# iden3/rapidsnark-old

Hardware: AMD Instinct MI355X
Metric: Groth16 proofs/sec (higher is better)
Workload: dtype i64 (v_mad_i64_i32 column sums over 9x29-bit signed limbs, BN254 Fr/Fq)

## Files before the change

rapidsnark-old_amd/csrc/kernels.hpp:

```cpp
#pragma once
#include <hip/hip_runtime.h>
#include <stdint.h>
#include "field.hpp"
#include "curve.hpp"

namespace zk {

void launch_fr_mul_vec(Fr *out, const Fr *a, const Fr *b, uint64_t n, hipStream_t s);
void launch_fq_mul_vec(Fq *out, const Fq *a, const Fq *b, uint64_t n, hipStream_t s);

struct CsrDev {
    const uint32_t *rowptr;
    const uint32_t *col;
    const Fr *val;
};
void launch_spmv_abc(Fr *a, Fr *b, Fr *c, CsrDev csr, const Fr *wtns, uint32_t n, hipStream_t s, uint32_t vectors = 1, uint64_t abc_stride = 0,
                     uint64_t wtns_stride = 0);
void launch_csr_build(uint32_t *rowptr, uint32_t *col, Fr *val, uint32_t *cursor, uint32_t *err, const uint8_t *records,
                      uint64_t nCoefs, uint32_t n, uint32_t nVars, uint32_t row_lo, uint32_t row_hi, hipStream_t s);
void launch_exclusive_scan_u32(uint32_t *out, const uint32_t *counts, uint32_t total, hipStream_t s);

struct TwEntry {
    uint32_t l[12];
};
// ... 23 lines not shown
void launch_ntt_build_tables(TwEntry *fwd, TwEntry *inv, Fr *coset, Fr *ninv, uint32_t logn, hipStream_t s);
#define NTT_FULL 0xffffffffu
void launch_ntt_dif_inverse(Fr *data, uint64_t stride_elems, uint32_t batch, const NttTables &t, hipStream_t s, uint32_t local_logn = NTT_FULL);
void launch_ntt_dit_forward(Fr *data, uint64_t stride_elems, uint32_t batch, const NttTables &t, hipStream_t s, const Fr *premul = nullptr,
                            uint32_t local_logn = NTT_FULL);
void launch_ntt_cross(bool inverse, const Fr *xb, uint64_t in_src_stride, uint64_t in_poly_stride, Fr *const out_base[8],
                      uint64_t out_poly_stride, uint64_t out_offset, uint32_t batch,
                      const NttTables &t, uint32_t log_shards, uint32_t rank, hipStream_t s);
void launch_chunk_scatter(Fr *const xb_of_gpu[8], const Fr *blockdata, uint32_t batch, uint32_t logn, uint32_t log_shards, uint32_t rank,
                          hipStream_t s);
void launch_chunk_pack(Fr *packed, const Fr *blockdata, uint32_t batch, uint32_t logn, uint32_t log_shards, hipStream_t s);
void launch_chunk_unpack(Fr *blockdata, const Fr *packed, uint32_t batch, uint32_t logn, uint32_t log_shards, hipStream_t s);
void launch_fr_to_internal(Fr *x, uint64_t n, int times, hipStream_t s);
void launch_fr_from_internal(Fr *x, uint64_t n, hipStream_t s);
void launch_fr_scale_by_table(Fr *data, uint64_t stride_elems, uint32_t batch, const Fr *table, uint64_t n, hipStream_t s);
void launch_fr_scale_const(Fr *data, const Fr *k, uint64_t n, hipStream_t s);
void launch_bitrev_permute(Fr *data, uint32_t logn, hipStream_t s);
void launch_abc_to_h(Fr *h, const Fr *a, const Fr *b, const Fr *c, uint64_t n, hipStream_t s, uint32_t vectors = 1, uint64_t abc_stride = 0);

struct MsmPlan {
    uint32_t c;
    uint32_t W;
    uint32_t nbuckets;
    uint32_t sets;
    uint32_t precomp;
    uint32_t batch;
    uint32_t batch_n;
};
MsmPlan make_msm_plan(uint64_t n, uint32_t window_bits, uint32_t precomp = 0, uint32_t batch = 1);
inline uint32_t msm_table_rows(const MsmPlan &p) { return p.precomp ? (p.W + p.precomp - 1) / p.precomp : 1u; }

struct MsmSortSizes {
    uint64_t counts_u32, starts_u32, offsets_u32, entries_u32;
    uint64_t codes_u32, lo_u16, val_u32, bin_counts_u32, bin_starts_u32;
};
struct MsmSortBufs {
    uint32_t *offsets, *entries;
    uint32_t *counts, *starts;
    uint32_t *codes, *val, *bin_counts, *bin_starts;
    uint16_t *lo;
};
MsmSortSizes msm_sort_sizes(uint64_t n, MsmPlan p);
uint32_t msm_scan_extra_words(uint32_t total);
void launch_msm_sort(const MsmSortBufs &b, const Fr *scalars, uint64_t n, MsmPlan p, hipStream_t s);
void launch_msm_precomp_g1(G1Affine *table, G1XYZZ *tmp, Fq *pref, uint64_t n, MsmPlan p, hipStream_t s);
void launch_msm_precomp_g2(G2Affine *table, G2XYZZ *tmp, Fq2 *pref, uint64_t n, MsmPlan p, hipStream_t s);
struct alignas(16) G1Acc {
    int32_t l[36];
};
struct alignas(16) G2Acc {
    int32_t l[72];
};
uint64_t msm_accum_workspace_slots(uint64_t max_entries);
struct AccumTail {
    hipStream_t stream = nullptr;
    hipEvent_t l1_done = nullptr;
    bool buckets_zeroed = false;
    uint32_t chunk_min = 0;
    uint32_t chunk_max = 0;
};
struct AccumBatch {
    uint32_t n;
    const void *points[3];
    uint32_t idx_min[3], idx_sub[3];
    uint64_t bucket_stride, ws_stride;
    uint32_t gather_mask;
};
void launch_msm_accum_g1_batch(G1Acc *buckets, const uint32_t *offsets, const uint32_t *entries, const AccumBatch &batch, uint32_t total_buckets,
                               uint64_t max_entries, G1Acc *ws_part, uint32_t *ws_key, uint32_t *ws_flag, hipStream_t s, hipEvent_t *ev = nullptr,
                               AccumTail tail = AccumTail());
void launch_msm_accum_g1(G1Acc *buckets, const uint32_t *offsets, const uint32_t *entries, const G1Affine *points,
                         uint32_t idx_min, uint32_t idx_sub, uint32_t total_buckets, uint64_t max_entries,
// ... 22 lines not shown
```

rapidsnark-old_amd/csrc/msm.hip:

```cpp
#include <stdlib.h>
#include "kernels.hpp"
#include "hipcheck.hpp"
#include "common.hpp"
#include "field29.hpp"
#include "curve29.hpp"
#include <string.h>

namespace zk {

#define REDUCE_CHUNK 16u
#define REDUCE_THREADS 256u

MsmPlan make_msm_plan(uint64_t n, uint32_t window_bits, uint32_t precomp, uint32_t batch) {
    if (precomp > 2) throw std::invalid_argument("table mode: 0 (as in the zkey), 1 (a row per window) or 2 (a row per second window)");
    MsmPlan p;
    uint32_t lg = 0;
    while ((1ull << (lg + 1)) <= n) lg++;
    uint32_t c = window_bits;
    if (precomp) {
        if (c == 0) {
            c = lg > 2 ? lg - 2 : 2;
            if (lg == 20) c = 19;
            if (lg == 21) c = 20;
            if (batch > 1) c++;
            if (c > 20) c = 20;
        }
        if (c > 22) c = 22;
    } else {
        if (c == 0) c = lg > 6 ? lg - 6 : 2;
        if (c > 16) c = 16;
    }
    if (c < 2) c = 2;
    p.c = c;
    p.W = (256 + c - 1) / c;
    {
        const uint32_t W255 = (255 + c - 1) / c;
        if (W255 < p.W) {
            const uint32_t sh = (W255 - 1) * c;
// ... 151 lines not shown
        int32_t w[36];
        load36(w, p->l);
        return unpack36(w);
    }
    __device__ __forceinline__ static void store(G1Acc *p, const XYZZ<R> &v) {
        int32_t w[36];
        pack36(w, v.x, v.y, v.zz, v.zzz);
        store36(p->l, w);
    }
    __device__ __forceinline__ static void store256(G1XYZZ *p, const XYZZ<R> &v) { store_xyzz_mont256(p, v); }
};
template <> struct LaneModel<Fq2> {
    static constexpr uint32_t LPE = 2;
    typedef Fq2s R;
    typedef G2Acc Mem;
    __device__ __forceinline__ static XYZZ<R> load(const G2Acc *p) {
        int32_t w[36];
        load36(w, p->l + 36 * (threadIdx.x & 1u));
        const XYZZ<Fq29> t = unpack36(w);
        return XYZZ<R>{R{t.x}, R{t.y}, R{t.zz}, R{t.zzz}};
    }
    __device__ __forceinline__ static void store(G2Acc *p, const XYZZ<R> &v) {
        int32_t w[36];
        pack36(w, v.x.v, v.y.v, v.zz.v, v.zzz.v);
        store36(p->l + 36 * (threadIdx.x & 1u), w);
    }
    __device__ __forceinline__ static void store256(G2XYZZ *p, const XYZZ<R> &v) {
        Fq *c = reinterpret_cast<Fq *>(p) + (threadIdx.x & 1u);
        Reg<Fq>::store256(c, v.x.v); Reg<Fq>::store256(c + 2, v.y.v); Reg<Fq>::store256(c + 4, v.zz.v); Reg<Fq>::store256(c + 6, v.zzz.v);
    }
};
#define ACCMEM typename LaneModel<F>::Mem

#define CODE32_ZERO 0x7FFFFFFFu
#ifndef SORT_THREADS
#define SORT_THREADS 1024u
#endif

__global__ __launch_bounds__(256) void k_msm_digits(uint32_t *digits, const Fr *scalars, uint64_t n, MsmPlan p) {
    ZK_CHAIN_PRIO();
    uint64_t st = (uint64_t)gridDim.x * blockDim.x;
    const uint32_t c = p.c, W = p.W;
    const uint32_t mask = (1u << c) - 1u, half = 1u << (c - 1);
    const uint32_t set_stride = p.precomp == 1 ? 0u : p.nbuckets, set_mask = p.precomp == 2 ? 1u : 0xffffffffu;
    for (uint64_t i = (uint64_t)blockIdx.x * blockDim.x + threadIdx.x; i < n; i += st) {
        Fr s = load_el(scalars + i);
        const uint32_t vec_base = p.batch > 1 ? (uint32_t)(i / p.batch_n) * p.nbuckets : 0u;
        for (int k = 0; k < 6; k++) {
            Fr d;
            u32 bw = 0;
#pragma unroll
            for (int j = 0; j < 8; j++) d.v[j] = subb(s.v[j], FrParams::P[j], bw);
            if (bw) break;
            s = d;
        }
        uint64_t buf = 0;
        uint32_t nb = 0, w = 0, carry = 0;
        auto emit = [&](uint32_t raw) {
            uint32_t d = raw + carry;
            const bool neg = d >= half;
            carry = neg ? 1u : 0u;
            uint32_t mag = neg ? (1u << c) - d : d;
            uint32_t code = mag ? ((mag - 1u + (w & set_mask) * set_stride + vec_base) | (neg ? 0x80000000u : 0u)) : CODE32_ZERO;
            digits[(uint64_t)w * n + i] = code;
            w++;
        };
#pragma unroll
        for (int k = 0; k < 8; k++) {
            buf |= (uint64_t)s.v[k] << nb;
            nb += 32;
            while (nb >= c && w + 1 < W) {
                emit((uint32_t)buf & mask);
                buf >>= c;
                nb -= c;
            }
        }
        emit((uint32_t)buf & mask);
    }
}

__global__ __launch_bounds__(256) void k_msm_compact_offsets(uint32_t *offsets, const uint32_t *starts, uint32_t total, uint32_t slices) {
    ZK_CHAIN_PRIO();
    uint32_t k = blockIdx.x * blockDim.x + threadIdx.x;
    if (k <= total) offsets[k] = starts[(uint64_t)k * slices];
}

#define BIN_MAX 256u

__global__ __launch_bounds__(SORT_THREADS) void k_bin_count(uint32_t *bin_counts, const uint32_t *codes, uint64_t total, uint32_t nbins,
                                                            uint32_t nblocks, uint32_t shift, uint32_t span) {
    ZK_CHAIN_PRIO();
    __shared__ uint32_t hist[BIN_MAX];
    if (threadIdx.x < BIN_MAX) hist[threadIdx.x] = 0;
    __syncthreads();
    const uint64_t base = (uint64_t)blockIdx.x * span;
    for (uint32_t k = threadIdx.x; k < span; k += SORT_THREADS) {
        uint64_t i = base + k;
        if (i < total) {
            uint32_t code = codes[i];
            if ((code & 0x7FFFFFFFu) != CODE32_ZERO) atomicAdd(&hist[(code & 0x7FFFFFFFu) >> shift], 1u);
        }
    }
    __syncthreads();
    if (threadIdx.x < nbins) bin_counts[(uint64_t)threadIdx.x * nblocks + blockIdx.x] = hist[threadIdx.x];
}

#define BIN_ITEMS 8u
__global__ __launch_bounds__(SORT_THREADS) void k_bin_scatter(uint16_t *lo, uint32_t *val, const uint32_t *bin_starts, const uint32_t *codes,
                                                              uint64_t total, uint32_t nbins, uint32_t nblocks, uint32_t shift, uint32_t span, uint64_t n,
                                                              uint32_t set_shift, uint32_t batch_n, uint32_t tstride) {
    ZK_CHAIN_PRIO();
    extern __shared__ uint32_t smem[];
    uint32_t *cnt = smem;
    uint32_t *gdelta = smem + BIN_MAX;
    uint32_t *st_dst = smem + 2 * BIN_MAX;
    uint32_t *st_val = st_dst + span;
    uint16_t *st_lo = (uint16_t *)(st_val + span);
    const uint32_t tid = threadIdx.x;
    if (tid < BIN_MAX) cnt[tid] = 0;
    __syncthreads();
    const uint64_t base = (uint64_t)blockIdx.x * span;
    const uint32_t lomask = (1u << shift) - 1u;
    const uint64_t w_base = tstride > 1 && n ? base / n : 0, r_base = tstride > 1 && n ? base - w_base * n : 0;
    uint32_t code[BIN_ITEMS], rank[BIN_ITEMS];
#pragma unroll
    for (uint32_t k = 0; k < BIN_ITEMS; k++) {
        uint64_t i = base + (uint64_t)k * SORT_THREADS + tid;
        code[k] = i < total ? codes[i] : CODE32_ZERO;
    }
#pragma unroll
    for (uint32_t k = 0; k < BIN_ITEMS; k++) {
        uint32_t mag = code[k] & 0x7FFFFFFFu;
        rank[k] = mag != CODE32_ZERO ? atomicAdd(&cnt[mag >> shift], 1u) : 0u;
    }
    __syncthreads();
    if (tid < 64) {
        uint32_t c0 = cnt[4 * tid], c1 = cnt[4 * tid + 1], c2 = cnt[4 * tid + 2], c3 = cnt[4 * tid + 3];
        uint32_t sum = c0 + c1 + c2 + c3, x = sum;
#pragma unroll
        for (int d = 1; d < 64; d <<= 1) {
            uint32_t y = __shfl_up(x, d);
            if (tid >= (uint32_t)d) x += y;
        }
        uint32_t off = x - sum;
        uint32_t o[4] = {off, off + c0, off + c0 + c1, off + c0 + c1 + c2};
#pragma unroll
        for (int q = 0; q < 4; q++) {
            uint32_t bin = 4 * tid + q;
            cnt[bin] = o[q];
            gdelta[bin] = bin < nbins ? bin_starts[(uint64_t)bin * nblocks + blockIdx.x] - o[q] : 0u;
        }
        if (tid == 63) smem[2 * BIN_MAX + 2 * span + span / 2] = x;
    }
    __syncthreads();
#pragma unroll
    for (uint32_t k = 0; k < BIN_ITEMS; k++) {
        uint32_t mag = code[k] & 0x7FFFFFFFu;
        if (mag != CODE32_ZERO) {
            uint32_t bin = mag >> shift, slot = cnt[bin] + rank[k];
            uint64_t i = base + (uint64_t)k * SORT_THREADS + tid - (uint64_t)(set_shift < 32 ? mag >> set_shift : 0u) * n;
            if (tstride > 1) {
                uint64_t w = w_base, r = r_base + (uint64_t)k * SORT_THREADS + tid;
                while (n && r >= n) { r -= n; w++; }
                i = (w / tstride) * n + r;
            }
            if (batch_n) {
                const uint64_t j = i / n, r = (i % n) % batch_n;
                i = j * batch_n + r;
            }
            st_dst[slot] = slot + gdelta[bin];
            st_val[slot] = (uint32_t)i | (code[k] & 0x80000000u);
            st_lo[slot] = (uint16_t)(mag & lomask);
        }
    }
    __syncthreads();
    const uint32_t kept = smem[2 * BIN_MAX + 2 * span + span / 2];
    for (uint32_t sidx = tid; sidx < kept; sidx += SORT_THREADS) {
        uint32_t d = st_dst[sidx];
        val[d] = st_val[sidx];
        lo[d] = st_lo[sidx];
    }
}

__device__ __forceinline__ bool bin_slice_of_block(uint32_t nbins, uint32_t slices, uint32_t &bin, uint32_t &slice) {
    const uint32_t xcd = blockIdx.x & 7u, k = blockIdx.x >> 3;
    bin = (k / slices) * 8u + xcd;
    slice = k % slices;
    return bin < nbins;
}

__global__ __launch_bounds__(SORT_THREADS) void k_bin_count_lds(uint32_t *counts, const uint16_t *lo, const uint32_t *bin_starts,
                                                                uint32_t nblocks, uint32_t buckets_per_bin, uint32_t nbins, uint32_t slices,
                                                                uint32_t total_buckets) {
    ZK_CHAIN_PRIO();
    extern __shared__ uint32_t hist[];
    uint32_t b, slice;
    if (!bin_slice_of_block(nbins, slices, b, slice)) return;
    const uint32_t first = b * buckets_per_bin, nb = total_buckets - first < buckets_per_bin ? total_buckets - first : buckets_per_bin;
    for (uint32_t k = threadIdx.x; k < nb; k += SORT_THREADS) hist[k] = 0;
    __syncthreads();
    const uint64_t bs = bin_starts[(uint64_t)b * nblocks], be = bin_starts[(uint64_t)(b + 1) * nblocks];
    const uint64_t len = be - bs, s0 = bs + len * slice / slices, s1 = bs + len * (slice + 1) / slices;
    for (uint64_t i = s0 + threadIdx.x; i < s1; i += SORT_THREADS) atomicAdd(&hist[lo[i]], 1u);
    __syncthreads();
    uint32_t *out = counts + (uint64_t)first * slices + slice;
    for (uint32_t k = threadIdx.x; k < nb; k += SORT_THREADS) out[(uint64_t)k * slices] = hist[k];
}

__global__ __launch_bounds__(SORT_THREADS) void k_bin_scatter_lds(uint32_t *entries, const uint32_t *starts, const uint16_t *lo,
                                                                  const uint32_t *val, const uint32_t *bin_starts, uint32_t nblocks,
                                                                  uint32_t buckets_per_bin, uint32_t nbins, uint32_t slices, uint32_t total_buckets) {
    ZK_CHAIN_PRIO();
    extern __shared__ uint32_t cursor[];
    uint32_t b, slice;
    if (!bin_slice_of_block(nbins, slices, b, slice)) return;
    const uint32_t first = b * buckets_per_bin, nb = total_buckets - first < buckets_per_bin ? total_buckets - first : buckets_per_bin;
    const uint32_t *in = starts + (uint64_t)first * slices + slice;
    for (uint32_t k = threadIdx.x; k < nb; k += SORT_THREADS) cursor[k] = in[(uint64_t)k * slices];
    __syncthreads();
    const uint64_t bs = bin_starts[(uint64_t)b * nblocks], be = bin_starts[(uint64_t)(b + 1) * nblocks];
    const uint64_t len = be - bs, s0 = bs + len * slice / slices, s1 = bs + len * (slice + 1) / slices;
    uint64_t i = s0 + threadIdx.x;
    for (; i + 3 * SORT_THREADS < s1; i += 4 * SORT_THREADS) {
        uint32_t k0 = lo[i], k1 = lo[i + SORT_THREADS], k2 = lo[i + 2 * SORT_THREADS], k3 = lo[i + 3 * SORT_THREADS];
        uint32_t v0 = val[i], v1 = val[i + SORT_THREADS], v2 = val[i + 2 * SORT_THREADS], v3 = val[i + 3 * SORT_THREADS];
        entries[atomicAdd(&cursor[k0], 1u)] = v0;
        entries[atomicAdd(&cursor[k1], 1u)] = v1;
        entries[atomicAdd(&cursor[k2], 1u)] = v2;
        entries[atomicAdd(&cursor[k3], 1u)] = v3;
    }
    for (; i < s1; i += SORT_THREADS) entries[atomicAdd(&cursor[lo[i]], 1u)] = val[i];
}

#define SCAN_BLOCK 1024u
#define SCAN_ELEMS 4096u
__device__ __forceinline__ uint32_t block_exclusive_scan(uint32_t v, uint32_t *lds, uint32_t &block_total) {
    const uint32_t tid = threadIdx.x, lane = tid & 63u, wave = tid >> 6;
    uint32_t x = v;
#pragma unroll
    for (int d = 1; d < 64; d <<= 1) {
        uint32_t y = __shfl_up(x, d);
        if (lane >= (uint32_t)d) x += y;
    }
    if (lane == 63) lds[wave] = x;
    __syncthreads();
    if (wave == 0) {
        uint32_t s = lane < (SCAN_BLOCK / 64) ? lds[lane] : 0;
#pragma unroll
        for (int d = 1; d < 16; d <<= 1) {
            uint32_t y = __shfl_up(s, d);
            if (lane >= (uint32_t)d) s += y;
// ... 15 lines not shown
    uint32_t sum = v[0] + v[1] + v[2] + v[3], bt;
    uint32_t ex = block_exclusive_scan(sum, lds, bt);
#pragma unroll
    for (int j = 0; j < 4; j++) {
        if (base + j < total) offsets[base + j] = ex;
        ex += v[j];
    }
    if (threadIdx.x == 0) block_sums[blockIdx.x] = bt;
}
__global__ __launch_bounds__(SCAN_BLOCK) void k_scan_sums(uint32_t *block_sums, uint32_t nblocks, uint32_t *grand_total) {
    ZK_CHAIN_PRIO();
    __shared__ uint32_t lds[SCAN_BLOCK / 64];
    __shared__ uint32_t carry_s;
    if (threadIdx.x == 0) carry_s = 0;
    __syncthreads();
    for (uint32_t base = 0; base < nblocks; base += SCAN_BLOCK) {
        uint32_t i = base + threadIdx.x;
        uint32_t v = i < nblocks ? block_sums[i] : 0, bt;
        uint32_t ex = block_exclusive_scan(v, lds, bt) + carry_s;
        if (i < nblocks) block_sums[i] = ex;
        __syncthreads();
        if (threadIdx.x == 0) carry_s += bt;
        __syncthreads();
    }
    if (threadIdx.x == 0) *grand_total = carry_s;
}
__global__ __launch_bounds__(SCAN_BLOCK) void k_scan_add(uint32_t *offsets, const uint32_t *block_sums, uint32_t total) {
    ZK_CHAIN_PRIO();
    const uint32_t base = blockIdx.x * SCAN_ELEMS + threadIdx.x * 4;
    const uint32_t add = block_sums[blockIdx.x];
#pragma unroll
    for (int j = 0; j < 4; j++)
        if (base + j < total) offsets[base + j] += add;
}

#ifndef STAGE_CAP
#define STAGE_CAP 8192u
#endif
static_assert(SCAN_BLOCK == 1024u && STAGE_CAP % SCAN_BLOCK == 0 && STAGE_CAP <= 65536u, "k_bin_scatter_staged: retune its LDS layout with SCAN_BLOCK / STAGE_CAP");
__global__ __launch_bounds__(SCAN_BLOCK) void k_bin_scatter_staged(uint32_t *entries, const uint32_t *starts, const uint16_t *lo, const uint32_t *val,
                                                                   const uint32_t *bin_starts, uint32_t nblocks, uint32_t buckets_per_bin, uint32_t nbins,
                                                                   uint32_t slices, uint32_t total_buckets) {
    ZK_CHAIN_PRIO();
    extern __shared__ uint32_t sm[];
    uint32_t b, slice;
    if (!bin_slice_of_block(nbins, slices, b, slice)) return;
    const uint32_t first = b * buckets_per_bin, nb = total_buckets - first < buckets_per_bin ? total_buckets - first : buckets_per_bin;
    uint32_t *loc = sm;
    uint32_t *gcur = sm + 2048;
    uint32_t *scan_lds = sm + 4096;
    uint32_t *sval = sm + 4096 + 16;
    uint16_t *slo = (uint16_t *)(sval + STAGE_CAP);
    const uint32_t tid = threadIdx.x;
    const uint32_t *in = starts + (uint64_t)first * slices + slice;
    for (uint32_t k = tid; k < 2048u; k += SCAN_BLOCK) gcur[k] = k < nb ? in[(uint64_t)k * slices] : 0u;
    const uint64_t bs = bin_starts[(uint64_t)b * nblocks], be = bin_starts[(uint64_t)(b + 1) * nblocks];
    const uint64_t len = be - bs, s0 = bs + len * slice / slices, s1 = bs + len * (slice + 1) / slices;
    constexpr uint32_t PER = STAGE_CAP / SCAN_BLOCK;
    for (uint64_t t0 = s0; t0 < s1; t0 += STAGE_CAP) {
        const uint32_t cnt = (uint32_t)(s1 - t0 < STAGE_CAP ? s1 - t0 : STAGE_CAP);
        loc[tid] = 0;
        loc[tid + SCAN_BLOCK] = 0;
        __syncthreads();
        uint32_t key[PER], v[PER], rank[PER];
#pragma unroll
        for (uint32_t k = 0; k < PER; k++) {
            const uint32_t p = k * SCAN_BLOCK + tid;
            key[k] = p < cnt ? lo[t0 + p] : 0xFFFFFFFFu;
            v[k] = p < cnt ? val[t0 + p] : 0u;
        }
#pragma unroll
        for (uint32_t k = 0; k < PER; k++) rank[k] = key[k] != 0xFFFFFFFFu ? atomicAdd(&loc[key[k]], 1u) : 0u;
        __syncthreads();
        const uint32_t c0 = loc[2 * tid], c1 = loc[2 * tid + 1];
        uint32_t total;
        const uint32_t ex = block_exclusive_scan(c0 + c1, scan_lds, total);
        __syncthreads();
        loc[2 * tid] = ex;
        loc[2 * tid + 1] = ex + c0;
        __syncthreads();
#pragma unroll
        for (uint32_t k = 0; k < PER; k++) {
            if (key[k] != 0xFFFFFFFFu) {
                const uint32_t pos = loc[key[k]] + rank[k];
                sval[pos] = v[k];
                slo[pos] = (uint16_t)key[k];
            }
        }
// ... 546 lines not shown
    return L >= 8u && (L / reduce_split_top(L)) % (2u * REDUCE_THREADS) == 0 && L / TREE_IN_MIN <= REDUCE_THREADS / 2u ? ch : 0u;
}

static inline uint64_t tree_points(uint64_t groups, uint64_t cnt) {
    uint64_t total = 0;
    for (;;) {
        total += groups * cnt;
        if (cnt == 1) break;
        cnt = (cnt + TREE_IN_MIN - 1) / TREE_IN_MIN;
    }
    return total + groups;
}
uint64_t msm_reduce_scratch_points(uint32_t n_msm, MsmPlan p) {
    if (reduce_bits_for(p)) return (uint64_t)n_msm * p.sets * (p.nbuckets / 128u + 1u) * BITS_RS;
    const uint64_t groups = (uint64_t)n_msm * p.sets;
    if (const uint32_t ch = reduce_split_for(p)) {
        const uint64_t L = p.nbuckets / ch;
        return groups * L + tree_points(groups, L / reduce_split_top((uint32_t)L) + L);
    }
    return tree_points(groups, p.nbuckets / reduce_chunk_for(p));
}

static void launch_scan(uint32_t *out, const uint32_t *counts, uint32_t total, hipStream_t s) {
    uint32_t nblocks = (total + SCAN_ELEMS - 1) / SCAN_ELEMS;
    uint32_t *block_sums = out + total + 1;
    ZK_LAUNCH(k_scan_local, dim3(nblocks), dim3(SCAN_BLOCK), 0, s, out, block_sums, counts, total);
    ZK_LAUNCH(k_scan_sums, dim3(1), dim3(SCAN_BLOCK), 0, s, block_sums, nblocks, out + total);
    ZK_LAUNCH(k_scan_add, dim3(nblocks), dim3(SCAN_BLOCK), 0, s, out, (const uint32_t *)block_sums, total);
}
uint32_t msm_scan_extra_words(uint32_t total) { return (total + SCAN_ELEMS - 1) / SCAN_ELEMS; }
void launch_exclusive_scan_u32(uint32_t *out, const uint32_t *counts, uint32_t total, hipStream_t s) { launch_scan(out, counts, total, s); }

#define BIN_SHIFT 11u
#define BIN_SLICES 32u
static inline uint32_t plan_total_buckets(MsmPlan p) { return p.sets * p.nbuckets; }
static inline uint32_t plan_bin_shift(MsmPlan p) {
    uint32_t sh = BIN_SHIFT;
    while (((plan_total_buckets(p) + (1u << sh) - 1) >> sh) > BIN_MAX) sh++;
    return sh;
}
static inline uint32_t plan_nbins(MsmPlan p) { uint32_t sh = plan_bin_shift(p); return (plan_total_buckets(p) + (1u << sh) - 1) >> sh; }
static inline uint32_t bin_span() { return BIN_ITEMS * SORT_THREADS; }
static inline uint32_t plan_bin_blocks(uint64_t n, MsmPlan p) { return (uint32_t)(((n ? n : 1) * p.W + bin_span() - 1) / bin_span()); }

MsmSortSizes msm_sort_sizes(uint64_t n, MsmPlan p) {
    MsmSortSizes z;
    memset(&z, 0, sizeof z);
    const uint64_t tb = plan_total_buckets(p), items = (n ? n : 1) * p.W;
    const uint64_t bb = (uint64_t)plan_nbins(p) * plan_bin_blocks(n, p);
    z.counts_u32 = tb * BIN_SLICES;
    z.starts_u32 = tb * BIN_SLICES + 1 + msm_scan_extra_words((uint32_t)(tb * BIN_SLICES));
    z.offsets_u32 = tb + 1;
    z.entries_u32 = items;
    z.codes_u32 = items;
    z.lo_u16 = items;
    z.val_u32 = items;
    z.bin_counts_u32 = bb;
    z.bin_starts_u32 = bb + 1 + msm_scan_extra_words((uint32_t)bb);
    return z;
}

static inline size_t bin_scatter_lds_bytes() { return (size_t)(2 * BIN_MAX + 2 * bin_span() + bin_span() / 2 + 1) * 4; }
static void sort_lds_attr() {
    static PerDeviceOnce attr;
    if (!attr.need()) return;
    ZK_HIP(hipFuncSetAttribute((const void *)k_bin_count_lds, hipFuncAttributeMaxDynamicSharedMemorySize, 160 * 1024));
    ZK_HIP(hipFuncSetAttribute((const void *)k_bin_scatter_lds, hipFuncAttributeMaxDynamicSharedMemorySize, 160 * 1024));
    ZK_HIP(hipFuncSetAttribute((const void *)k_bin_scatter, hipFuncAttributeMaxDynamicSharedMemorySize, 160 * 1024));
    ZK_HIP(hipFuncSetAttribute((const void *)k_bin_scatter_staged, hipFuncAttributeMaxDynamicSharedMemorySize, 160 * 1024));
    attr.done();
}

void launch_msm_sort(const MsmSortBufs &b, const Fr *scalars, uint64_t n, MsmPlan p, hipStream_t s) {
    const uint32_t tb = plan_total_buckets(p);
    sort_lds_attr();
    uint64_t g = (n + 255) / 256;
    if (g > 8192) g = 8192;
    const uint32_t sh = plan_bin_shift(p), nbins = plan_nbins(p), nblocks = plan_bin_blocks(n, p);
    uint32_t slices = BIN_SLICES;
    {
        const uint64_t per_bin = (n * p.W) / (nbins ? nbins : 1);
        while (slices > 4u && per_bin / slices < STAGE_CAP * 3u / 4u) slices >>= 1;
    }
    const uint32_t bpb = tb < (1u << sh) ? tb : (1u << sh);
    const uint64_t total = n * p.W;
    const size_t lds = (size_t)bpb * 4;
    const uint32_t grid2 = ((nbins + 7u) / 8u) * 8u * slices;
    const uint32_t set_shift = p.precomp ? 32u : p.c - 1u;
    if (n) ZK_LAUNCH(k_msm_digits, dim3((uint32_t)g), dim3(256), 0, s, b.codes, scalars, n, p);
    ZK_LAUNCH(k_bin_count, dim3(nblocks), dim3(SORT_THREADS), 0, s, b.bin_counts, (const uint32_t *)b.codes, total, nbins, nblocks, sh, bin_span());
    launch_scan(b.bin_starts, b.bin_counts, nbins * nblocks, s);
    ZK_LAUNCH(k_bin_scatter, dim3(nblocks), dim3(SORT_THREADS), bin_scatter_lds_bytes(), s, b.lo, b.val, (const uint32_t *)b.bin_starts,
                       (const uint32_t *)b.codes, total, nbins, nblocks, sh, bin_span(), n, set_shift, p.batch > 1 ? p.batch_n : 0u, p.precomp);
    ZK_LAUNCH(k_bin_count_lds, dim3(grid2), dim3(SORT_THREADS), lds, s, b.counts, (const uint16_t *)b.lo,
                       (const uint32_t *)b.bin_starts, nblocks, bpb, nbins, slices, tb);
    launch_scan(b.starts, b.counts, tb * slices, s);
    static const bool direct = probe_env("ZKHIP_SORT_DIRECT") != nullptr;
    if (bpb <= 2048u && SORT_THREADS == SCAN_BLOCK && !direct)
        ZK_LAUNCH(k_bin_scatter_staged, dim3(grid2), dim3(SCAN_BLOCK), (size_t)(4096 + 16 + STAGE_CAP) * 4 + (size_t)STAGE_CAP * 2, s, b.entries,
                           (const uint32_t *)b.starts, (const uint16_t *)b.lo, (const uint32_t *)b.val, (const uint32_t *)b.bin_starts, nblocks, bpb, nbins,
                           slices, tb);
    else
        ZK_LAUNCH(k_bin_scatter_lds, dim3(grid2), dim3(SORT_THREADS), lds, s, b.entries, (const uint32_t *)b.starts,
                           (const uint16_t *)b.lo, (const uint32_t *)b.val, (const uint32_t *)b.bin_starts, nblocks, bpb, nbins, slices, tb);
    ZK_LAUNCH(k_msm_compact_offsets, dim3((tb + 256) / 256), dim3(256), 0, s, b.offsets, (const uint32_t *)b.starts, tb, slices);
    ZK_LAUNCH_OK("msm sort");
}

template <class F>
__global__ __launch_bounds__(128) void k_precomp_walk(XYZZ<F> *tmp, const Affine<F> *pts, uint64_t n, uint32_t c, uint32_t W) {
    uint64_t i = (uint64_t)blockIdx.x * blockDim.x + threadIdx.x;
    if (i >= n) return;
    typedef REGF FR;
    XYZZ<FR> acc = XYZZ<FR>::from_affine(load_affine(pts + i));
    for (uint32_t j = 1; j < W; j++) {
        for (uint32_t k = 0; k < c; k++) acc = dbl(acc);
        store_xyzz(tmp + (uint64_t)(j - 1) * n + i, acc);
    }
}
template <class F>
__global__ __launch_bounds__(64) void k_precomp_normalize(Affine<F> *out, const XYZZ<F> *tmp, F *pref, uint64_t total) {
    const uint64_t lo = ((uint64_t)blockIdx.x * blockDim.x + threadIdx.x) * 64;
    if (lo >= total) return;
    const uint64_t hi = lo + 64 < total ? lo + 64 : total;
    typedef REGF FR;
    FR acc = FR::one();
    for (uint64_t i = lo; i < hi; i++) {
        Reg<F>::store(pref + i, acc);
        FR t = FR::mul(Reg<F>::load(&tmp[i].zz), Reg<F>::load(&tmp[i].zzz));
        if (!t.is_zero()) acc = FR::mul(acc, t);
    }
    FR inv = FR::inv(acc);
    for (uint64_t i = hi; i-- > lo;) {
        FR zz = Reg<F>::load(&tmp[i].zz), zzz = Reg<F>::load(&tmp[i].zzz);
        FR t = FR::mul(zz, zzz);
        if (t.is_zero()) {
            Reg<F>::store(&out[i].x, FR::zero());
            Reg<F>::store(&out[i].y, FR::zero());
// ... 204 lines not shown
```

rapidsnark-old_amd/csrc/prover_internal.hpp:

```cpp
#pragma once
#include <hip/hip_runtime.h>
#include <string.h>
#include <stdio.h>
#include <stdlib.h>
#include <chrono>
#include <sys/random.h>
#include <string>
#include <vector>
#include <atomic>
#include <condition_variable>
#include <deque>
#include <map>
#include <mutex>
#include <thread>
#include <memory>
#include <stdexcept>
#include <exception>
#include <functional>

#include "../../include/zkhip.h"
#include "common.hpp"
#include "hipcheck.hpp"
#include "kernels.hpp"
#include "tail_pool.hpp"
// ... 63 lines not shown
            }
            const uint8_t *from = (const uint8_t *)src + off;
            uint8_t *to = pin[k];
            const size_t nt = 4, per = (len / nt + 4095) & ~(size_t)4095;
            std::vector<std::thread> th;
            for (size_t t = 1; t < nt; t++) {
                const size_t lo = t * per, hi = lo + per < len ? lo + per : len;
                if (lo < hi) th.emplace_back([=] { memcpy(to + lo, from + lo, hi - lo); });
            }
            memcpy(to, from, per < len ? per : len);
            for (auto &t : th) t.join();
            HIP_TRY(hipMemcpyAsync((uint8_t *)dst + off, to, len, hipMemcpyHostToDevice, s));
            HIP_TRY(hipEventRecord(done[k], s));
        }
    }
};

struct Slice {
    uint64_t lo, hi;
    uint64_t size() const { return hi - lo; }
};
inline Slice shard_slice(uint64_t n, uint32_t idx, uint32_t cnt) {
    uint64_t per = (n + cnt - 1) / cnt;
    uint64_t lo = per * idx, hi = lo + per;
    if (lo > n) lo = n;
    if (hi > n) hi = n;
    return Slice{lo, hi};
}

struct SortBufs {
    MsmPlan plan;
    uint64_t n = 0;
    DevBuf<uint16_t> lo;
    DevBuf<uint32_t> counts, starts, offsets, entries, codes, val, bin_counts, bin_starts;
    uint32_t total_buckets() const { return plan.sets * plan.nbuckets; }
    uint64_t max_entries() const { return (n ? n : 1) * plan.W; }
    void alloc(uint64_t n_, uint32_t window_bits, uint32_t precomp = 0, uint32_t batch = 1) {
        plan = make_msm_plan(n_ ? n_ : 1, window_bits, precomp, batch);
        n = n_ * (batch > 1 ? batch : 1);
        if ((n ? n : 1) * plan.W >= (1ull << 32)) throw std::invalid_argument("MSM too large: n * windows >= 2^32 sort entries");
        if ((n ? n : 1) * msm_table_rows(plan) >= (1ull << 31)) throw std::invalid_argument("MSM too large: table rows >= 2^31");
        MsmSortSizes z = msm_sort_sizes(n, plan);
        lo.alloc(z.lo_u16);
        counts.alloc(z.counts_u32);
        starts.alloc(z.starts_u32);
        offsets.alloc(z.offsets_u32);
        entries.alloc(z.entries_u32);
        codes.alloc(z.codes_u32);
        val.alloc(z.val_u32);
        bin_counts.alloc(z.bin_counts_u32);
        bin_starts.alloc(z.bin_starts_u32);
    }
    void release() {
        lo.release(); counts.release(); starts.release(); offsets.release(); entries.release();
        codes.release(); val.release(); bin_counts.release(); bin_starts.release();
        n = 0; ran = false;
    }
    size_t bytes() const {
        return lo.bytes() + counts.bytes() + starts.bytes() + offsets.bytes() + entries.bytes() + codes.bytes() + val.bytes()
             + bin_counts.bytes() + bin_starts.bytes();
    }
    bool ran = false;
    void run(const Fr *scalars, hipStream_t s) {
        static const bool skip = probe_env("ZKHIP_PROBE_SKIP_SORT") != nullptr;
        if (skip && ran) return;
        ran = true;
        MsmSortBufs b{offsets.p, entries.p, counts.p, starts.p, codes.p, val.p, bin_counts.p, bin_starts.p, lo.p};
        launch_msm_sort(b, scalars, n, plan, s);
    }
};


}
using namespace zkp;

struct StageJob {
    uint8_t *dst;
    const uint8_t *src;
    size_t bytes;
};

struct zk_prover {
    int device = 0;
    uint32_t flags = 0;
    uint32_t nVars = 0, nPublic = 0, domainSize = 0, logn = 0;
    uint64_t nCoefs = 0;
    uint32_t shard_index = 0, shard_count = 1;
    uint8_t vk_alpha1[64], vk_beta1[64], vk_beta2[128], vk_delta1[64], vk_delta2[128];
    hipStream_t stream = nullptr, stream2 = nullptr;
    std::mutex mtx, cmtx, sync_mtx;

    DevBuf<uint32_t> csr_rowptr, csr_col;
    DevBuf<Fr> csr_val;
    DevBuf<TwEntry> tw_fwd, tw_inv;
    DevBuf<Fr> tw_coset, tw_ninv;
    NttPair pair;
    Slice sv, sh;
    uint32_t c_idx_min = 0;
    bool precomp = false;
    uint32_t table_mode = 0;
// ... 243 lines not shown
```

Measured before the change: 30.30.

## Fuse scalar digit recoding into MSM bin passes and restructure bucket cursor scan

Removes the separate digit-recoding kernel and its codes buffer. The bin count and bin scatter kernels now load scalars and recompute the signed digits on the fly, with one scalar per thread. The per-bucket slice counts are laid out contiguously per bin, and a new per-bin cursor kernel replaces the global scan plus offsets compaction kernel. The lo histogram pass now uses 128-bit vector loads and BIN_SLICES drops from 32 to 16. This trades a write and re-read of n*W codes for recomputing the recoding twice, once in count and once in scatter, with double atomics in scatter.

```diff
diff --git a/rapidsnark-old_amd/csrc/kernels.hpp b/rapidsnark-old_amd/csrc/kernels.hpp
--- a/rapidsnark-old_amd/csrc/kernels.hpp
+++ b/rapidsnark-old_amd/csrc/kernels.hpp
@@ -79,12 +79,12 @@
 
 struct MsmSortSizes {
     uint64_t counts_u32, starts_u32, offsets_u32, entries_u32;
-    uint64_t codes_u32, lo_u16, val_u32, bin_counts_u32, bin_starts_u32;
+    uint64_t lo_u16, val_u32, bin_counts_u32, bin_starts_u32;
 };
 struct MsmSortBufs {
     uint32_t *offsets, *entries;
     uint32_t *counts, *starts;
-    uint32_t *codes, *val, *bin_counts, *bin_starts;
+    uint32_t *val, *bin_counts, *bin_starts;
     uint16_t *lo;
 };
 MsmSortSizes msm_sort_sizes(uint64_t n, MsmPlan p);
diff --git a/rapidsnark-old_amd/csrc/msm.hip b/rapidsnark-old_amd/csrc/msm.hip
--- a/rapidsnark-old_amd/csrc/msm.hip
+++ b/rapidsnark-old_amd/csrc/msm.hip
@@ -4,6 +4,7 @@
 #include "common.hpp"
 #include "field29.hpp"
 #include "curve29.hpp"
+#include "msm_digits.hpp"
 #include <string.h>
 
 namespace zk {
@@ -221,107 +222,72 @@
 };
 #define ACCMEM typename LaneModel<F>::Mem
 
-#define CODE32_ZERO 0x7FFFFFFFu
 #ifndef SORT_THREADS
 #define SORT_THREADS 1024u
 #endif
 
-__global__ __launch_bounds__(256) void k_msm_digits(uint32_t *digits, const Fr *scalars, uint64_t n, MsmPlan p) {
-    ZK_CHAIN_PRIO();
-    uint64_t st = (uint64_t)gridDim.x * blockDim.x;
-    const uint32_t c = p.c, W = p.W;
-    const uint32_t mask = (1u << c) - 1u, half = 1u << (c - 1);
-    const uint32_t set_stride = p.precomp == 1 ? 0u : p.nbuckets, set_mask = p.precomp == 2 ? 1u : 0xffffffffu;
-    for (uint64_t i = (uint64_t)blockIdx.x * blockDim.x + threadIdx.x; i < n; i += st) {
-        Fr s = load_el(scalars + i);
-        const uint32_t vec_base = p.batch > 1 ? (uint32_t)(i / p.batch_n) * p.nbuckets : 0u;
-        for (int k = 0; k < 6; k++) {
-            Fr d;
-            u32 bw = 0;
-#pragma unroll
-            for (int j = 0; j < 8; j++) d.v[j] = subb(s.v[j], FrParams::P[j], bw);
-            if (bw) break;
-            s = d;
-        }
-        uint64_t buf = 0;
-        uint32_t nb = 0, w = 0, carry = 0;
-        auto emit = [&](uint32_t raw) {
-            uint32_t d = raw + carry;
-            const bool neg = d >= half;
-            carry = neg ? 1u : 0u;
-            uint32_t mag = neg ? (1u << c) - d : d;
-            uint32_t code = mag ? ((mag - 1u + (w & set_mask) * set_stride + vec_base) | (neg ? 0x80000000u : 0u)) : CODE32_ZERO;
-            digits[(uint64_t)w * n + i] = code;
-            w++;
-        };
-#pragma unroll
-        for (int k = 0; k < 8; k++) {
-            buf |= (uint64_t)s.v[k] << nb;
-            nb += 32;
-            while (nb >= c && w + 1 < W) {
-                emit((uint32_t)buf & mask);
-                buf >>= c;
-                nb -= c;
-            }
-        }
-        emit((uint32_t)buf & mask);
-    }
-}
-
-__global__ __launch_bounds__(256) void k_msm_compact_offsets(uint32_t *offsets, const uint32_t *starts, uint32_t total, uint32_t slices) {
-    ZK_CHAIN_PRIO();
-    uint32_t k = blockIdx.x * blockDim.x + threadIdx.x;
-    if (k <= total) offsets[k] = starts[(uint64_t)k * slices];
+struct BinScalars {
+    const Fr *scalars;
+    uint64_t n;
+    MsmDigitKeys keys;
+    uint32_t per_block;
+    uint32_t nbuckets;
+    uint32_t batch_n;
+    uint32_t row_stride;
+    uint32_t row_shift;
+};
+__device__ __forceinline__ bool bin_load_scalar(const BinScalars &a, uint32_t s[8], uint32_t &row, uint32_t &vec_base) {
+    const uint64_t i = (uint64_t)blockIdx.x * a.per_block + threadIdx.x;
+    if (threadIdx.x >= a.per_block || i >= a.n) return false;
+    const Fr v = load_el(a.scalars + i);
+#pragma unroll
+    for (int j = 0; j < 8; j++) s[j] = v.v[j];
+    msm_scalar_below_r(s);
+    const uint32_t vec = a.batch_n ? (uint32_t)i / a.batch_n : 0u;
+    row = (uint32_t)i - vec * a.batch_n;
+    vec_base = vec * a.nbuckets;
+    return true;
 }
 
 #define BIN_MAX 256u
 
-__global__ __launch_bounds__(SORT_THREADS) void k_bin_count(uint32_t *bin_counts, const uint32_t *codes, uint64_t total, uint32_t nbins,
-                                                            uint32_t nblocks, uint32_t shift, uint32_t span) {
+#ifndef BIN_THREADS
+#define BIN_THREADS 512u
+#define BIN_ITEMS_CAP 7168u
+#endif
+__global__ __launch_bounds__(BIN_THREADS) void k_bin_count(uint32_t *bin_counts, BinScalars a, uint32_t nbins, uint32_t nblocks, uint32_t shift) {
     ZK_CHAIN_PRIO();
     __shared__ uint32_t hist[BIN_MAX];
     if (threadIdx.x < BIN_MAX) hist[threadIdx.x] = 0;
     __syncthreads();
-    const uint64_t base = (uint64_t)blockIdx.x * span;
-    for (uint32_t k = threadIdx.x; k < span; k += SORT_THREADS) {
-        uint64_t i = base + k;
-        if (i < total) {
-            uint32_t code = codes[i];
-            if ((code & 0x7FFFFFFFu) != CODE32_ZERO) atomicAdd(&hist[(code & 0x7FFFFFFFu) >> shift], 1u);
-        }
-    }
+    uint32_t s[8], row, vec_base;
+    if (bin_load_scalar(a, s, row, vec_base))
+        msm_recode_below_r(s, a.keys, vec_base, [&](uint32_t, uint32_t code) {
+            if (code != CODE32_ZERO) atomicAdd(&hist[(code & 0x7FFFFFFFu) >> shift], 1u);
+        });
     __syncthreads();
     if (threadIdx.x < nbins) bin_counts[(uint64_t)threadIdx.x * nblocks + blockIdx.x] = hist[threadIdx.x];
 }
 
-#define BIN_ITEMS 8u
-__global__ __launch_bounds__(SORT_THREADS) void k_bin_scatter(uint16_t *lo, uint32_t *val, const uint32_t *bin_starts, const uint32_t *codes,
-                                                              uint64_t total, uint32_t nbins, uint32_t nblocks, uint32_t shift, uint32_t span, uint64_t n,
-                                                              uint32_t set_shift, uint32_t batch_n, uint32_t tstride) {
+__global__ __launch_bounds__(BIN_THREADS) void k_bin_scatter(uint16_t *lo, uint32_t *val, const uint32_t *bin_starts, BinScalars a, uint32_t nbins,
+                                                             uint32_t nblocks, uint32_t shift, uint32_t cap) {
     ZK_CHAIN_PRIO();
     extern __shared__ uint32_t smem[];
     uint32_t *cnt = smem;
     uint32_t *gdelta = smem + BIN_MAX;
     uint32_t *st_dst = smem + 2 * BIN_MAX;
-    uint32_t *st_val = st_dst + span;
-    uint16_t *st_lo = (uint16_t *)(st_val + span);
+    uint32_t *st_val = st_dst + cap;
+    uint16_t *st_lo = (uint16_t *)(st_val + cap);
     const uint32_t tid = threadIdx.x;
     if (tid < BIN_MAX) cnt[tid] = 0;
     __syncthreads();
-    const uint64_t base = (uint64_t)blockIdx.x * span;
     const uint32_t lomask = (1u << shift) - 1u;
-    const uint64_t w_base = tstride > 1 && n ? base / n : 0, r_base = tstride > 1 && n ? base - w_base * n : 0;
-    uint32_t code[BIN_ITEMS], rank[BIN_ITEMS];
-#pragma unroll
-    for (uint32_t k = 0; k < BIN_ITEMS; k++) {
-        uint64_t i = base + (uint64_t)k * SORT_THREADS + tid;
-        code[k] = i < total ? codes[i] : CODE32_ZERO;
-    }
-#pragma unroll
-    for (uint32_t k = 0; k < BIN_ITEMS; k++) {
-        uint32_t mag = code[k] & 0x7FFFFFFFu;
-        rank[k] = mag != CODE32_ZERO ? atomicAdd(&cnt[mag >> shift], 1u) : 0u;
-    }
+    uint32_t s[8], row = 0, vec_base = 0;
+    const bool have = bin_load_scalar(a, s, row, vec_base);
+    if (have)
+        msm_recode_below_r(s, a.keys, vec_base, [&](uint32_t, uint32_t code) {
+            if (code != CODE32_ZERO) atomicAdd(&cnt[(code & 0x7FFFFFFFu) >> shift], 1u);
+        });
     __syncthreads();
     if (tid < 64) {
         uint32_t c0 = cnt[4 * tid], c1 = cnt[4 * tid + 1], c2 = cnt[4 * tid + 2], c3 = cnt[4 * tid + 3];
@@ -339,32 +305,21 @@
             cnt[bin] = o[q];
             gdelta[bin] = bin < nbins ? bin_starts[(uint64_t)bin * nblocks + blockIdx.x] - o[q] : 0u;
         }
-        if (tid == 63) smem[2 * BIN_MAX + 2 * span + span / 2] = x;
-    }
-    __syncthreads();
-#pragma unroll
-    for (uint32_t k = 0; k < BIN_ITEMS; k++) {
-        uint32_t mag = code[k] & 0x7FFFFFFFu;
-        if (mag != CODE32_ZERO) {
-            uint32_t bin = mag >> shift, slot = cnt[bin] + rank[k];
-            uint64_t i = base + (uint64_t)k * SORT_THREADS + tid - (uint64_t)(set_shift < 32 ? mag >> set_shift : 0u) * n;
-            if (tstride > 1) {
-                uint64_t w = w_base, r = r_base + (uint64_t)k * SORT_THREADS + tid;
-                while (n && r >= n) { r -= n; w++; }
-                i = (w / tstride) * n + r;
+        if (tid == 63) smem[2 * BIN_MAX + 2 * cap + cap / 2] = x;
+    }
+    __syncthreads();
+    if (have)
+        msm_recode_below_r(s, a.keys, vec_base, [&](uint32_t w, uint32_t code) {
+            if (code != CODE32_ZERO) {
+                const uint32_t mag = code & 0x7FFFFFFFu, bin = mag >> shift, slot = atomicAdd(&cnt[bin], 1u);
+                st_dst[slot] = slot + gdelta[bin];
+                st_val[slot] = ((w >> a.row_shift) * a.row_stride + row) | (code & 0x80000000u);
+                st_lo[slot] = (uint16_t)(mag & lomask);
             }
-            if (batch_n) {
-                const uint64_t j = i / n, r = (i % n) % batch_n;
-                i = j * batch_n + r;
-            }
-            st_dst[slot] = slot + gdelta[bin];
-            st_val[slot] = (uint32_t)i | (code[k] & 0x80000000u);
-            st_lo[slot] = (uint16_t)(mag & lomask);
-        }
-    }
-    __syncthreads();
-    const uint32_t kept = smem[2 * BIN_MAX + 2 * span + span / 2];
-    for (uint32_t sidx = tid; sidx < kept; sidx += SORT_THREADS) {
+        });
+    __syncthreads();
+    const uint32_t kept = smem[2 * BIN_MAX + 2 * cap + cap / 2];
+    for (uint32_t sidx = tid; sidx < kept; sidx += BIN_THREADS) {
         uint32_t d = st_dst[sidx];
         val[d] = st_val[sidx];
         lo[d] = st_lo[sidx];
@@ -390,10 +345,25 @@
     __syncthreads();
     const uint64_t bs = bin_starts[(uint64_t)b * nblocks], be = bin_starts[(uint64_t)(b + 1) * nblocks];
     const uint64_t len = be - bs, s0 = bs + len * slice / slices, s1 = bs + len * (slice + 1) / slices;
-    for (uint64_t i = s0 + threadIdx.x; i < s1; i += SORT_THREADS) atomicAdd(&hist[lo[i]], 1u);
-    __syncthreads();
-    uint32_t *out = counts + (uint64_t)first * slices + slice;
-    for (uint32_t k = threadIdx.x; k < nb; k += SORT_THREADS) out[(uint64_t)k * slices] = hist[k];
+    const uint64_t up = (s0 + 7u) & ~(uint64_t)7u, a0 = up < s1 ? up : s1, nvec = (s1 - a0) >> 3, a1 = a0 + (nvec << 3);
+    if (s0 + threadIdx.x < a0) atomicAdd(&hist[lo[s0 + threadIdx.x]], 1u);
+    if (a1 + threadIdx.x < s1) atomicAdd(&hist[lo[a1 + threadIdx.x]], 1u);
+    const uint4 *q = reinterpret_cast<const uint4 *>(lo + a0);
+    auto count8 = [&](const uint4 &x) {
+        atomicAdd(&hist[x.x & 0xffffu], 1u); atomicAdd(&hist[x.x >> 16], 1u);
+        atomicAdd(&hist[x.y & 0xffffu], 1u); atomicAdd(&hist[x.y >> 16], 1u);
+        atomicAdd(&hist[x.z & 0xffffu], 1u); atomicAdd(&hist[x.z >> 16], 1u);
+        atomicAdd(&hist[x.w & 0xffffu], 1u); atomicAdd(&hist[x.w >> 16], 1u);
+    };
+    uint64_t v = threadIdx.x;
+    for (; v + 3 * SORT_THREADS < nvec; v += 4 * SORT_THREADS) {
+        const uint4 x0 = q[v], x1 = q[v + SORT_THREADS], x2 = q[v + 2 * SORT_THREADS], x3 = q[v + 3 * SORT_THREADS];
+        count8(x0); count8(x1); count8(x2); count8(x3);
+    }
+    for (; v < nvec; v += SORT_THREADS) count8(q[v]);
+    __syncthreads();
+    uint32_t *out = counts + ((uint64_t)b * slices + slice) * buckets_per_bin;
+    for (uint32_t k = threadIdx.x; k < nb; k += SORT_THREADS) out[k] = hist[k];
 }
 
 __global__ __launch_bounds__(SORT_THREADS) void k_bin_scatter_lds(uint32_t *entries, const uint32_t *starts, const uint16_t *lo,
@@ -404,8 +374,8 @@
     uint32_t b, slice;
     if (!bin_slice_of_block(nbins, slices, b, slice)) return;
     const uint32_t first = b * buckets_per_bin, nb = total_buckets - first < buckets_per_bin ? total_buckets - first : buckets_per_bin;
-    const uint32_t *in = starts + (uint64_t)first * slices + slice;
-    for (uint32_t k = threadIdx.x; k < nb; k += SORT_THREADS) cursor[k] = in[(uint64_t)k * slices];
+    const uint32_t *in = starts + ((uint64_t)b * slices + slice) * buckets_per_bin;
+    for (uint32_t k = threadIdx.x; k < nb; k += SORT_THREADS) cursor[k] = in[k];
     __syncthreads();
     const uint64_t bs = bin_starts[(uint64_t)b * nblocks], be = bin_starts[(uint64_t)(b + 1) * nblocks];
     const uint64_t len = be - bs, s0 = bs + len * slice / slices, s1 = bs + len * (slice + 1) / slices;
@@ -487,6 +457,40 @@
 #pragma unroll
     for (int j = 0; j < 4; j++)
         if (base + j < total) offsets[base + j] += add;
+}
+
+#ifndef BIN_SLICES
+#define BIN_SLICES 16u
+#endif
+__global__ __launch_bounds__(SCAN_BLOCK) void k_bin_cursors(uint32_t *starts, uint32_t *offsets, const uint32_t *counts, const uint32_t *bin_starts,
+                                                            uint32_t nblocks, uint32_t buckets_per_bin, uint32_t nbins, uint32_t slices,
+                                                            uint32_t total_buckets) {
+    ZK_CHAIN_PRIO();
+    __shared__ uint32_t lds[SCAN_BLOCK / 64];
+    const uint32_t b = blockIdx.x, tid = threadIdx.x;
+    const uint32_t first = b * buckets_per_bin, nb = total_buckets - first < buckets_per_bin ? total_buckets - first : buckets_per_bin;
+    const uint64_t at = (uint64_t)b * slices * buckets_per_bin;
+    uint32_t run = bin_starts[(uint64_t)b * nblocks];
+    for (uint32_t k0 = 0; k0 < nb; k0 += SCAN_BLOCK) {
+        const uint32_t k = k0 + tid;
+        uint32_t pre[BIN_SLICES], sum = 0;
+#pragma unroll
+        for (uint32_t sl = 0; sl < BIN_SLICES; sl++) {
+            pre[sl] = sum;
+            if (sl < slices && k < nb) sum += counts[at + (uint64_t)sl * buckets_per_bin + k];
+        }
+        uint32_t chunk_total;
+        const uint32_t bstart = run + block_exclusive_scan(sum, lds, chunk_total);
+        if (k < nb) {
+            offsets[first + k] = bstart;
+#pragma unroll
+            for (uint32_t sl = 0; sl < BIN_SLICES; sl++)
+                if (sl < slices) starts[at + (uint64_t)sl * buckets_per_bin + k] = bstart + pre[sl];
+        }
+        run += chunk_total;
+        __syncthreads();
+    }
+    if (b == nbins - 1 && tid == 0) offsets[total_buckets] = bin_starts[(uint64_t)nbins * nblocks];
 }
 
 #ifndef STAGE_CAP
@@ -507,8 +511,8 @@
     uint32_t *sval = sm + 4096 + 16;
     uint16_t *slo = (uint16_t *)(sval + STAGE_CAP);
     const uint32_t tid = threadIdx.x;
-    const uint32_t *in = starts + (uint64_t)first * slices + slice;
-    for (uint32_t k = tid; k < 2048u; k += SCAN_BLOCK) gcur[k] = k < nb ? in[(uint64_t)k * slices] : 0u;
+    const uint32_t *in = starts + ((uint64_t)b * slices + slice) * buckets_per_bin;
+    for (uint32_t k = tid; k < 2048u; k += SCAN_BLOCK) gcur[k] = k < nb ? in[k] : 0u;
     const uint64_t bs = bin_starts[(uint64_t)b * nblocks], be = bin_starts[(uint64_t)(b + 1) * nblocks];
     const uint64_t len = be - bs, s0 = bs + len * slice / slices, s1 = bs + len * (slice + 1) / slices;
     constexpr uint32_t PER = STAGE_CAP / SCAN_BLOCK;
@@ -1121,7 +1125,6 @@
 void launch_exclusive_scan_u32(uint32_t *out, const uint32_t *counts, uint32_t total, hipStream_t s) { launch_scan(out, counts, total, s); }
 
 #define BIN_SHIFT 11u
-#define BIN_SLICES 32u
 static inline uint32_t plan_total_buckets(MsmPlan p) { return p.sets * p.nbuckets; }
 static inline uint32_t plan_bin_shift(MsmPlan p) {
     uint32_t sh = BIN_SHIFT;
@@ -1129,19 +1132,22 @@
     return sh;
 }
 static inline uint32_t plan_nbins(MsmPlan p) { uint32_t sh = plan_bin_shift(p); return (plan_total_buckets(p) + (1u << sh) - 1) >> sh; }
-static inline uint32_t bin_span() { return BIN_ITEMS * SORT_THREADS; }
-static inline uint32_t plan_bin_blocks(uint64_t n, MsmPlan p) { return (uint32_t)(((n ? n : 1) * p.W + bin_span() - 1) / bin_span()); }
+static inline uint32_t plan_bin_scalars(MsmPlan p) {
+    const uint32_t s = BIN_ITEMS_CAP / p.W;
+    return s < BIN_THREADS ? s : BIN_THREADS;
+}
+static inline uint32_t plan_bin_blocks(uint64_t n, MsmPlan p) { return (uint32_t)(((n ? n : 1) + plan_bin_scalars(p) - 1) / plan_bin_scalars(p)); }
 
 MsmSortSizes msm_sort_sizes(uint64_t n, MsmPlan p) {
     MsmSortSizes z;
     memset(&z, 0, sizeof z);
     const uint64_t tb = plan_total_buckets(p), items = (n ? n : 1) * p.W;
     const uint64_t bb = (uint64_t)plan_nbins(p) * plan_bin_blocks(n, p);
-    z.counts_u32 = tb * BIN_SLICES;
-    z.starts_u32 = tb * BIN_SLICES + 1 + msm_scan_extra_words((uint32_t)(tb * BIN_SLICES));
+    const uint64_t bpb = tb < (1ull << plan_bin_shift(p)) ? tb : 1ull << plan_bin_shift(p);
+    z.counts_u32 = (uint64_t)plan_nbins(p) * BIN_SLICES * bpb;
+    z.starts_u32 = z.counts_u32;
     z.offsets_u32 = tb + 1;
     z.entries_u32 = items;
-    z.codes_u32 = items;
     z.lo_u16 = items;
     z.val_u32 = items;
     z.bin_counts_u32 = bb;
@@ -1149,7 +1155,8 @@
     return z;
 }
 
-static inline size_t bin_scatter_lds_bytes() { return (size_t)(2 * BIN_MAX + 2 * bin_span() + bin_span() / 2 + 1) * 4; }
+static inline uint32_t bin_scatter_cap(MsmPlan p) { return (plan_bin_scalars(p) * p.W + 1u) & ~1u; }
+static inline size_t bin_scatter_lds_bytes(uint32_t cap) { return (size_t)(2 * BIN_MAX + 2 * cap + cap / 2 + 1) * 4; }
 static void sort_lds_attr() {
     static PerDeviceOnce attr;
     if (!attr.need()) return;
@@ -1163,8 +1170,6 @@
 void launch_msm_sort(const MsmSortBufs &b, const Fr *scalars, uint64_t n, MsmPlan p, hipStream_t s) {
     const uint32_t tb = plan_total_buckets(p);
     sort_lds_attr();
-    uint64_t g = (n + 255) / 256;
-    if (g > 8192) g = 8192;
     const uint32_t sh = plan_bin_shift(p), nbins = plan_nbins(p), nblocks = plan_bin_blocks(n, p);
     uint32_t slices = BIN_SLICES;
     {
@@ -1172,18 +1177,19 @@
         while (slices > 4u && per_bin / slices < STAGE_CAP * 3u / 4u) slices >>= 1;
     }
     const uint32_t bpb = tb < (1u << sh) ? tb : (1u << sh);
-    const uint64_t total = n * p.W;
     const size_t lds = (size_t)bpb * 4;
     const uint32_t grid2 = ((nbins + 7u) / 8u) * 8u * slices;
-    const uint32_t set_shift = p.precomp ? 32u : p.c - 1u;
-    if (n) ZK_LAUNCH(k_msm_digits, dim3((uint32_t)g), dim3(256), 0, s, b.codes, scalars, n, p);
-    ZK_LAUNCH(k_bin_count, dim3(nblocks), dim3(SORT_THREADS), 0, s, b.bin_counts, (const uint32_t *)b.codes, total, nbins, nblocks, sh, bin_span());
+    BinScalars a{scalars, n, msm_digit_keys(p.c, p.W, p.nbuckets, p.precomp), plan_bin_scalars(p), p.nbuckets, p.batch > 1 ? p.batch_n : 0u,
+                 p.precomp ? (p.batch > 1 ? p.batch_n : (uint32_t)n) : 0u, p.precomp == 2 ? 1u : 0u};
+    const uint32_t cap = bin_scatter_cap(p);
+    ZK_LAUNCH(k_bin_count, dim3(nblocks), dim3(BIN_THREADS), 0, s, b.bin_counts, a, nbins, nblocks, sh);
     launch_scan(b.bin_starts, b.bin_counts, nbins * nblocks, s);
-    ZK_LAUNCH(k_bin_scatter, dim3(nblocks), dim3(SORT_THREADS), bin_scatter_lds_bytes(), s, b.lo, b.val, (const uint32_t *)b.bin_starts,
-                       (const uint32_t *)b.codes, total, nbins, nblocks, sh, bin_span(), n, set_shift, p.batch > 1 ? p.batch_n : 0u, p.precomp);
+    ZK_LAUNCH(k_bin_scatter, dim3(nblocks), dim3(BIN_THREADS), bin_scatter_lds_bytes(cap), s, b.lo, b.val, (const uint32_t *)b.bin_starts, a, nbins,
+                       nblocks, sh, cap);
     ZK_LAUNCH(k_bin_count_lds, dim3(grid2), dim3(SORT_THREADS), lds, s, b.counts, (const uint16_t *)b.lo,
                        (const uint32_t *)b.bin_starts, nblocks, bpb, nbins, slices, tb);
-    launch_scan(b.starts, b.counts, tb * slices, s);
+    ZK_LAUNCH(k_bin_cursors, dim3(nbins), dim3(SCAN_BLOCK), 0, s, b.starts, b.offsets, (const uint32_t *)b.counts, (const uint32_t *)b.bin_starts, nblocks, bpb,
+                       nbins, slices, tb);
     static const bool direct = probe_env("ZKHIP_SORT_DIRECT") != nullptr;
     if (bpb <= 2048u && SORT_THREADS == SCAN_BLOCK && !direct)
         ZK_LAUNCH(k_bin_scatter_staged, dim3(grid2), dim3(SCAN_BLOCK), (size_t)(4096 + 16 + STAGE_CAP) * 4 + (size_t)STAGE_CAP * 2, s, b.entries,
@@ -1192,7 +1198,6 @@
     else
         ZK_LAUNCH(k_bin_scatter_lds, dim3(grid2), dim3(SORT_THREADS), lds, s, b.entries, (const uint32_t *)b.starts,
                            (const uint16_t *)b.lo, (const uint32_t *)b.val, (const uint32_t *)b.bin_starts, nblocks, bpb, nbins, slices, tb);
-    ZK_LAUNCH(k_msm_compact_offsets, dim3((tb + 256) / 256), dim3(256), 0, s, b.offsets, (const uint32_t *)b.starts, tb, slices);
     ZK_LAUNCH_OK("msm sort");
 }
 
diff --git a/rapidsnark-old_amd/csrc/msm_digits.hpp b/rapidsnark-old_amd/csrc/msm_digits.hpp
--- /dev/null
+++ b/rapidsnark-old_amd/csrc/msm_digits.hpp
@@ -0,0 +1,69 @@
+#pragma once
+#include "field.hpp"
+
+namespace zk {
+
+#define CODE32_ZERO 0x7FFFFFFFu
+
+struct MsmDigitKeys {
+    u32 c, W;
+    u32 set_stride, set_mask;
+};
+ZK_HD MsmDigitKeys msm_digit_keys(u32 c, u32 W, u32 nbuckets, u32 precomp) {
+    MsmDigitKeys k;
+    k.c = c;
+    k.W = W;
+    k.set_stride = precomp == 1 ? 0u : nbuckets;
+    k.set_mask = precomp == 2 ? 1u : 0xffffffffu;
+    return k;
+}
+
+ZK_HD void msm_scalar_below_r(u32 s[8]) {
+    for (int k = 0; k < 6; k++) {
+        u32 d[8];
+        u32 bw = 0;
+#pragma unroll
+        for (int j = 0; j < 8; j++) d[j] = subb(s[j], FrParams::P[j], bw);
+        if (bw) break;
+#pragma unroll
+        for (int j = 0; j < 8; j++) s[j] = d[j];
+    }
+}
+
+template <class Emit>
+ZK_HD void msm_recode_below_r(const u32 s[8], const MsmDigitKeys &p, u32 vec_base, Emit &&emit) {
+    const u32 c = p.c, W = p.W;
+    const u32 mask = (1u << c) - 1u, half = 1u << (c - 1);
+    u64 buf = 0;
+    u32 nb = 0, w = 0, carry = 0;
+    auto digit = [&](u32 raw) {
+        const u32 d = raw + carry;
+        const bool neg = d >= half;
+        carry = neg ? 1u : 0u;
+        const u32 mag = neg ? (1u << c) - d : d;
+        emit(w, mag ? ((mag - 1u + (w & p.set_mask) * p.set_stride + vec_base) | (neg ? 0x80000000u : 0u)) : CODE32_ZERO);
+        w++;
+    };
+#pragma unroll
+    for (int k = 0; k < 8; k++) {
+        buf |= (u64)s[k] << nb;
+        nb += 32;
+        while (nb >= c && w + 1 < W) {
+            digit((u32)buf & mask);
+            buf >>= c;
+            nb -= c;
+        }
+    }
+    digit((u32)buf & mask);
+}
+
+template <class Emit>
+ZK_HD void msm_recode(const u32 scalar[8], const MsmDigitKeys &p, u32 vec_base, Emit &&emit) {
+    u32 s[8];
+#pragma unroll
+    for (int j = 0; j < 8; j++) s[j] = scalar[j];
+    msm_scalar_below_r(s);
+    msm_recode_below_r(s, p, vec_base, emit);
+}
+
+}
diff --git a/rapidsnark-old_amd/csrc/prover_internal.hpp b/rapidsnark-old_amd/csrc/prover_internal.hpp
--- a/rapidsnark-old_amd/csrc/prover_internal.hpp
+++ b/rapidsnark-old_amd/csrc/prover_internal.hpp
@@ -119,7 +119,7 @@
     MsmPlan plan;
     uint64_t n = 0;
     DevBuf<uint16_t> lo;
-    DevBuf<uint32_t> counts, starts, offsets, entries, codes, val, bin_counts, bin_starts;
+    DevBuf<uint32_t> counts, starts, offsets, entries, val, bin_counts, bin_starts;
     uint32_t total_buckets() const { return plan.sets * plan.nbuckets; }
     uint64_t max_entries() const { return (n ? n : 1) * plan.W; }
     void alloc(uint64_t n_, uint32_t window_bits, uint32_t precomp = 0, uint32_t batch = 1) {
@@ -133,18 +133,17 @@
         starts.alloc(z.starts_u32);
         offsets.alloc(z.offsets_u32);
         entries.alloc(z.entries_u32);
-        codes.alloc(z.codes_u32);
         val.alloc(z.val_u32);
         bin_counts.alloc(z.bin_counts_u32);
         bin_starts.alloc(z.bin_starts_u32);
     }
     void release() {
         lo.release(); counts.release(); starts.release(); offsets.release(); entries.release();
-        codes.release(); val.release(); bin_counts.release(); bin_starts.release();
+        val.release(); bin_counts.release(); bin_starts.release();
         n = 0; ran = false;
     }
     size_t bytes() const {
-        return lo.bytes() + counts.bytes() + starts.bytes() + offsets.bytes() + entries.bytes() + codes.bytes() + val.bytes()
+        return lo.bytes() + counts.bytes() + starts.bytes() + offsets.bytes() + entries.bytes() + val.bytes()
              + bin_counts.bytes() + bin_starts.bytes();
     }
     bool ran = false;
@@ -152,7 +151,7 @@
         static const bool skip = probe_env("ZKHIP_PROBE_SKIP_SORT") != nullptr;
         if (skip && ran) return;
         ran = true;
-        MsmSortBufs b{offsets.p, entries.p, counts.p, starts.p, codes.p, val.p, bin_counts.p, bin_starts.p, lo.p};
+        MsmSortBufs b{offsets.p, entries.p, counts.p, starts.p, val.p, bin_counts.p, bin_starts.p, lo.p};
         launch_msm_sort(b, scalars, n, plan, s);
     }
 };
```

Result: no change. 30.41 (median of 3 runs) (+0.4%).
